# gmh14/tssplat

Measured on AMD Instinct MI355X. Metric: tetrahedra/sec (energy fwd+bwd), higher is better.
Workload: dtype f32

## Files before the change

include/tssplat_amd.h:

```cpp
#ifndef TSSPLAT_AMD_H
#define TSSPLAT_AMD_H

#include <stdint.h>

#ifdef __cplusplus
extern "C" {
#endif

typedef struct tsamd_handle tsamd_handle;

typedef enum tsamd_status {
    TSAMD_OK = 0,
    TSAMD_ERR_INVALID_ARGUMENT = 1,
    TSAMD_ERR_BAD_MESH = 2,
    TSAMD_ERR_NO_DEVICE = 3,
    TSAMD_ERR_HIP = 4,
    TSAMD_ERR_IO = 5,
    TSAMD_ERR_TILING = 6,
    TSAMD_ERR_HOST_ONLY = 7
} tsamd_status;

typedef struct tsamd_options {
    int32_t struct_size;
    int32_t device;
// ... 16 lines not shown
    int64_t total_slots;
    int64_t total_tile_vertices;
    int64_t shared_vertex_copies;
    int64_t finish_vertices;
    int64_t device_bytes;
    int32_t max_slots, max_tile_vertices, block_threads, lds_bytes;
    int32_t slots_per_thread;
    int32_t n_planes;
} tsamd_plan_info;

typedef struct tsamd_tile_view {
    int32_t n_slots, n_owned, s_pad, n_verts, n_excl;
    int64_t stage_off;
    int32_t n_rows;
    int32_t rec_base;
    const uint32_t *planes;
    const uint16_t *row_start;
    const int32_t *gvid;
    const int32_t *vdst;
    const int32_t *slot_tet;
    const float *rest;
} tsamd_tile_view;

const char *tsamd_last_error(void);
const char *tsamd_version(void);
#define TSAMD_ABI_VERSION 3
int32_t tsamd_abi_version(void);

int tsamd_create(const float *rest_xyz, int64_t n_vertices, const int32_t *tets, int64_t n_tets,
                 const tsamd_options *options, tsamd_handle **out);
int tsamd_create_from_veg(const char *path, const tsamd_options *options, tsamd_handle **out);
int tsamd_create_with_operator(const float *rest_xyz, int64_t n_vertices, const int32_t *tets, int64_t n_tets,
                               const int64_t *op_rowptr, const int32_t *op_col, const double *op_val,
                               const tsamd_options *options, tsamd_handle **out);
void tsamd_destroy(tsamd_handle *h);

int64_t tsamd_num_vertices(const tsamd_handle *h);
int64_t tsamd_num_tets(const tsamd_handle *h);
int tsamd_get_plan_info(const tsamd_handle *h, tsamd_plan_info *out);
int tsamd_get_tile(const tsamd_handle *h, int64_t tile, tsamd_tile_view *out);
int tsamd_get_finish_lists(const tsamd_handle *h, int64_t *n_finish, const int32_t **vid,
                           const int32_t **off, const int32_t **idx);
int tsamd_get_adjacency(const tsamd_handle *h, const int32_t **nbr);

int tsamd_forward(tsamd_handle *h, const float *x_dev, float c1, float c2, int order,
                  void *stream, float *energy_dev);
int tsamd_backward(tsamd_handle *h, const float *x_dev, const float *grad_out_dev, float c1, float c2,
                   int order, void *stream, float *grad_dev);
int tsamd_forward_backward(tsamd_handle *h, const float *x_dev, const float *grad_out_dev, float c1,
                           float c2, int order, void *stream, float *energy_dev, float *grad_dev);
int tsamd_evaluate_dev_coef(tsamd_handle *h, const float *x_dev, const float *grad_out_dev, const float *coef_dev,
                            int order, void *stream, float *energy_dev, float *grad_dev);
typedef struct tsamd_graph tsamd_graph;
int tsamd_graph_create(tsamd_handle *h, const float *x_dev, const float *grad_out_dev, int order, float *energy_dev,
                       float *grad_dev, tsamd_graph **out);
int tsamd_graph_launch(tsamd_graph *graph, float c1, float c2, void *stream);
int tsamd_graph_launch_to(tsamd_graph *graph, float c1, float c2, void *stream, float *energy_copy_dev, float *grad_dev);
void tsamd_graph_destroy(tsamd_graph *graph);

typedef struct tsamd_train_loop tsamd_train_loop;
int64_t tsamd_train_loop_workspace_bytes(int32_t n_iters);
int tsamd_train_loop_create(tsamd_handle *h, float *param_dev, float *grad_dev, float *g1_dev, float *g2_dev, float *energy_ring_dev,
                            void *workspace_dev, int32_t n_iters, tsamd_train_loop **out);
// ... 92 lines not shown
```

tssplat_amd/_capi.py:

```python
from __future__ import annotations

import ctypes as C
import os

from . import _build

_lib = None


class TsamdError(RuntimeError):

    def __init__(self, code: int, message: str):
        super().__init__(f"tssplat_amd error {code}: {message}")
        self.code = code


class Options(C.Structure):
    _fields_ = [
        ("struct_size", C.c_int32),
        ("device", C.c_int32),
        ("lds_budget_bytes", C.c_int32),
        ("max_threads", C.c_int32),
        ("target_owned", C.c_int32),
        ("lane_search_sweeps", C.c_int32),
# ... 8 lines not shown

class PlanInfo(C.Structure):
    _fields_ = [
        ("n_vertices", C.c_int64), ("n_tets", C.c_int64), ("n_tiles", C.c_int64),
        ("n_components", C.c_int64), ("total_slots", C.c_int64), ("total_tile_vertices", C.c_int64),
        ("shared_vertex_copies", C.c_int64), ("finish_vertices", C.c_int64), ("device_bytes", C.c_int64),
        ("max_slots", C.c_int32), ("max_tile_vertices", C.c_int32), ("block_threads", C.c_int32),
        ("lds_bytes", C.c_int32), ("slots_per_thread", C.c_int32), ("n_planes", C.c_int32),
    ]

    def as_dict(self) -> dict:
        return {k: int(getattr(self, k)) for k, _ in self._fields_}


class TileView(C.Structure):
    _fields_ = [
        ("n_slots", C.c_int32), ("n_owned", C.c_int32), ("s_pad", C.c_int32), ("n_verts", C.c_int32),
        ("n_excl", C.c_int32), ("stage_off", C.c_int64), ("n_rows", C.c_int32), ("rec_base", C.c_int32),
        ("planes", C.POINTER(C.c_uint32)), ("row_start", C.POINTER(C.c_uint16)),
        ("gvid", C.POINTER(C.c_int32)), ("vdst", C.POINTER(C.c_int32)), ("slot_tet", C.POINTER(C.c_int32)), ("rest", C.POINTER(C.c_float)),
    ]


ABI_VERSION = 3

SIGNATURES = {
    "tsamd_last_error": (C.c_char_p, []),
    "tsamd_version": (C.c_char_p, []),
    "tsamd_abi_version": (C.c_int32, []),
    "tsamd_create": (C.c_int, [C.c_void_p, C.c_int64, C.c_void_p, C.c_int64, C.POINTER(Options), C.POINTER(C.c_void_p)]),
    "tsamd_create_with_operator": (C.c_int, [C.c_void_p, C.c_int64, C.c_void_p, C.c_int64, C.c_void_p, C.c_void_p, C.c_void_p,
                                             C.POINTER(Options), C.POINTER(C.c_void_p)]),
    "tsamd_create_from_veg": (C.c_int, [C.c_char_p, C.POINTER(Options), C.POINTER(C.c_void_p)]),
    "tsamd_destroy": (None, [C.c_void_p]),
    "tsamd_num_vertices": (C.c_int64, [C.c_void_p]),
    "tsamd_num_tets": (C.c_int64, [C.c_void_p]),
    "tsamd_get_plan_info": (C.c_int, [C.c_void_p, C.POINTER(PlanInfo)]),
    "tsamd_get_tile": (C.c_int, [C.c_void_p, C.c_int64, C.POINTER(TileView)]),
    "tsamd_get_finish_lists": (C.c_int, [C.c_void_p, C.POINTER(C.c_int64), C.POINTER(C.POINTER(C.c_int32)),
                                         C.POINTER(C.POINTER(C.c_int32)), C.POINTER(C.POINTER(C.c_int32))]),
    "tsamd_get_adjacency": (C.c_int, [C.c_void_p, C.POINTER(C.POINTER(C.c_int32))]),
    "tsamd_forward": (C.c_int, [C.c_void_p, C.c_void_p, C.c_float, C.c_float, C.c_int, C.c_void_p, C.c_void_p]),
    "tsamd_backward": (C.c_int, [C.c_void_p, C.c_void_p, C.c_void_p, C.c_float, C.c_float, C.c_int, C.c_void_p,
                                 C.c_void_p]),
    "tsamd_forward_backward": (C.c_int, [C.c_void_p, C.c_void_p, C.c_void_p, C.c_float, C.c_float, C.c_int,
                                         C.c_void_p, C.c_void_p, C.c_void_p]),
    "tsamd_evaluate_dev_coef": (C.c_int, [C.c_void_p, C.c_void_p, C.c_void_p, C.c_void_p, C.c_int, C.c_void_p, C.c_void_p,
                                          C.c_void_p]),
    "tsamd_graph_create": (C.c_int, [C.c_void_p, C.c_void_p, C.c_void_p, C.c_int, C.c_void_p, C.c_void_p, C.POINTER(C.c_void_p)]),
    "tsamd_graph_launch": (C.c_int, [C.c_void_p, C.c_float, C.c_float, C.c_void_p]),
    "tsamd_graph_launch_to": (C.c_int, [C.c_void_p, C.c_float, C.c_float, C.c_void_p, C.c_void_p, C.c_void_p]),
    "tsamd_graph_destroy": (None, [C.c_void_p]),
    "tsamd_read_energy_terms": (C.c_int, [C.c_void_p, C.c_void_p, C.POINTER(C.c_double)]),
    "tsamd_set_timing": (C.c_int, [C.c_void_p, C.c_int]),
    "tsamd_get_timing": (C.c_int, [C.c_void_p, C.POINTER(C.c_double), C.POINTER(C.c_double), C.POINTER(C.c_int64)]),
    "tsamd_scale": (C.c_int, [C.c_void_p, C.c_void_p, C.c_void_p, C.c_int64, C.c_void_p]),
    "tsamd_adam_uniform_step": (C.c_int, [C.c_void_p, C.c_void_p, C.c_void_p, C.c_void_p, C.c_int64, C.c_float, C.c_float,
                                        C.c_float, C.c_int64, C.c_float, C.c_void_p, C.c_void_p]),
    "tsamd_grad_limit_workspace_bytes": (C.c_int64, []),
    "tsamd_grad_limit": (C.c_int, [C.c_void_p, C.c_int64, C.c_float, C.c_float, C.c_void_p, C.c_void_p]),
    "tsamd_train_loop_workspace_bytes": (C.c_int64, [C.c_int32]),
# ... 125 lines not shown
```

tssplat_amd/csrc/capi.cpp:

```cpp
#include "../../include/tssplat_amd.h"

#include <hip/hip_runtime_api.h>

#include <algorithm>
#include <cmath>
#include <cstdio>
#include <cstdlib>
#include <cstring>
#include <new>
#include <string>
#include <thread>
#include <vector>

#include "capi_common.h"
#include "kernels.h"
#include "plan.h"

namespace {

thread_local std::string g_err;

int fail(int code, const std::string &msg)
{
    g_err = msg;
// ... 340 lines not shown
    if (!h || !out) return fail(TSAMD_ERR_INVALID_ARGUMENT, "null argument");
    const tsamd::Plan &P = h->plan;
    if (tile < 0 || tile >= int64_t(P.tiles.size())) return fail(TSAMD_ERR_INVALID_ARGUMENT, "tile out of range");
    const tsamd::TileDesc &d = P.tiles[size_t(tile)];
    out->n_slots = d.n_slots;
    out->n_owned = d.n_owned;
    out->s_pad = d.s_pad;
    out->n_verts = d.n_verts;
    out->n_excl = d.n_excl;
    out->stage_off = d.stage_off;
    out->n_rows = d.n_rows;
    out->rec_base = d.rec_base;
    out->planes = P.blob.data() + d.blob_off / 4;
    out->row_start = reinterpret_cast<const uint16_t *>(reinterpret_cast<const uint8_t *>(out->planes) + tsamd::tile_rowtab_offset(P.n_planes, d.s_pad));
    out->gvid = P.gvid.data() + d.vert_off;
    out->vdst = P.vdst.data() + d.vert_off;
    out->slot_tet = P.slot_tet.data() + P.slot_base[size_t(tile)];
    out->rest = P.n_planes == tsamd::kPlanesRebuild
                    ? reinterpret_cast<const float *>(reinterpret_cast<const uint8_t *>(out->planes) + tsamd::tile_rest_offset(P.n_planes, d.s_pad))
                    : nullptr;
    return TSAMD_OK;
}

int tsamd_get_finish_lists(const tsamd_handle *h, int64_t *n_finish, const int32_t **vid, const int32_t **off,
                           const int32_t **idx)
{
    if (!h || !n_finish || !vid || !off || !idx) return fail(TSAMD_ERR_INVALID_ARGUMENT, "null argument");
    *n_finish = int64_t(h->plan.fin_vid.size());
    *vid = h->plan.fin_vid.data();
    *off = h->plan.fin_off.data();
    *idx = h->plan.fin_idx.data();
    return TSAMD_OK;
}

int tsamd_get_adjacency(const tsamd_handle *h, const int32_t **nbr)
{
    if (!h || !nbr) return fail(TSAMD_ERR_INVALID_ARGUMENT, "null argument");
    *nbr = h->plan.nbr.data();
    return TSAMD_OK;
}

int tsamd_forward(tsamd_handle *h, const float *x_dev, float c1, float c2, int order, void *stream,
                  float *energy_dev)
{
    if (!energy_dev) return fail(TSAMD_ERR_INVALID_ARGUMENT, "energy_dev is null");
    return evaluate(h, x_dev, nullptr, c1, c2, order, stream, energy_dev, nullptr);
// ... 221 lines not shown
```

tssplat_amd/csrc/partition.cpp:

```cpp
#include "partition.h"

#include <algorithm>
#include <cmath>

namespace tsamd {
namespace {

constexpr int kLloydIters = 12;
constexpr int kLloydFull = 4;
constexpr int kCandidates = 8;
constexpr int kImproveSweeps = 6;
constexpr int kConnectProbe = 512;
constexpr int64_t kMaxIncidence = int64_t(1) << 23;

inline int64_t copies(int64_t c) { return (c + kMaxRank - 1) / kMaxRank; }

struct Part {
    const Limits &lim;
    int64_t cnt = 0, nv = 0, k = 0;
    std::vector<int32_t> nb;
    std::vector<int32_t> lv;
    std::vector<double> x;
    std::vector<int32_t> part;
    std::vector<int64_t> owned, slots, verts;
    std::vector<int32_t> inc;
    std::vector<int32_t> mark, queue;
    int32_t stamp = 0;

    explicit Part(const Limits &l) : lim(l) {}

    int64_t cost(int64_t p) const { return kPartSlotWeight * slots[size_t(p)] + verts[size_t(p)]; }
    bool fits(int64_t p) const { return lim.fits(slots[size_t(p)], verts[size_t(p)]); }

    void seed(int32_t *idx, int64_t n, int64_t kk, int32_t &next)
    {
        if (kk <= 1) {
            for (int64_t i = 0; i < n; ++i) part[size_t(idx[i])] = next;
            ++next;
            return;
        }
        double lo[3], hi[3];
        for (int d = 0; d < 3; ++d) {
            lo[d] = std::numeric_limits<double>::max();
            hi[d] = -std::numeric_limits<double>::max();
        }
        for (int64_t i = 0; i < n; ++i)
            for (int d = 0; d < 3; ++d) {
                lo[d] = std::min(lo[d], x[3 * size_t(idx[i]) + d]);
                hi[d] = std::max(hi[d], x[3 * size_t(idx[i]) + d]);
            }
        int ax = 0;
        for (int d = 1; d < 3; ++d)
            if (hi[d] - lo[d] > hi[ax] - lo[ax]) ax = d;
        const int64_t k1 = kk / 2;
// ... 5 lines not shown
        seed(idx, mid, k1, next);
        seed(idx + mid, n - mid, kk - k1, next);
    }

    void count_slots(std::vector<int64_t> &s) const
    {
        s.assign(size_t(k), 0);
        for (int64_t q = 0; q < cnt; ++q) {
            const int32_t pq = part[size_t(q)];
            ++s[size_t(pq)];
            int32_t seen[4];
            int ns = 0;
            for (int f = 0; f < 4; ++f) {
                const int32_t r = nb[4 * size_t(q) + f];
                if (r < 0) continue;
                const int32_t pr = part[size_t(r)];
                if (pr == pq || std::find(seen, seen + ns, pr) != seen + ns) continue;
                seen[ns++] = pr;
                ++s[size_t(pr)];
            }
        }
    }

    void lloyd()
    {
        const size_t K = static_cast<size_t>(k);
        std::vector<double> c(3 * K, 0.0), w(K, 0.0), d2c(K);
        std::vector<int64_t> n_in(K), s;
        std::vector<int32_t> cand(K * kCandidates), order(K), next(static_cast<size_t>(cnt));
        const int nc = int(std::min<int64_t>(k, kCandidates));
        for (int it = 0; it < kLloydIters; ++it) {
            std::fill(n_in.begin(), n_in.end(), 0);
            std::vector<double> sum(3 * size_t(k), 0.0);
            for (int64_t e = 0; e < cnt; ++e) {
                const int32_t p = part[size_t(e)];
                ++n_in[size_t(p)];
                for (int d = 0; d < 3; ++d) sum[3 * size_t(p) + d] += x[3 * size_t(e) + d];
            }
            for (int64_t p = 0; p < k; ++p)
                if (n_in[size_t(p)] > 0)
                    for (int d = 0; d < 3; ++d) c[3 * size_t(p) + d] = sum[3 * size_t(p) + d] / double(n_in[size_t(p)]);
            count_slots(s);
            double r2 = 0.0;
            for (int64_t e = 0; e < cnt; ++e) {
                const int32_t p = part[size_t(e)];
                for (int d = 0; d < 3; ++d) {
                    const double t = x[3 * size_t(e) + d] - c[3 * size_t(p) + d];
                    r2 += t * t;
                }
            }
            r2 /= double(std::max<int64_t>(1, cnt));
            int64_t s_sum = 0, live = 0;
            for (int64_t p = 0; p < k; ++p)
                if (n_in[size_t(p)] > 0) {
                    s_sum += s[size_t(p)];
                    ++live;
                }
            const double s_mean = double(s_sum) / double(std::max<int64_t>(1, live));
            for (int64_t p = 0; p < k; ++p) w[size_t(p)] += 0.5 * r2 * (s_mean - double(s[size_t(p)])) / s_mean;
            for (int64_t p = 0; p < k; ++p) {
                for (int64_t q = 0; q < k; ++q) {
                    double d = 0.0;
                    for (int dd = 0; dd < 3; ++dd) {
                        const double t = c[3 * size_t(q) + dd] - c[3 * size_t(p) + dd];
                        d += t * t;
// ... 8 lines not shown
            }
            for (int64_t e = 0; e < cnt; ++e) {
                const int32_t p = part[size_t(e)];
                next[size_t(e)] = p;
                if (it >= kLloydFull && in_cell(int32_t(e), p) == faces(int32_t(e))) continue;
                int32_t best = p;
                double best_d = std::numeric_limits<double>::max();
                for (int j = 0; j < nc; ++j) {
                    const int32_t q = cand[size_t(p) * kCandidates + size_t(j)];
                    double d = -w[size_t(q)];
                    for (int dd = 0; dd < 3; ++dd) {
                        const double t = x[3 * size_t(e) + dd] - c[3 * size_t(q) + dd];
                        d += t * t;
                    }
                    if (d < best_d || (d == best_d && q < best)) {
                        best_d = d;
                        best = q;
                    }
                }
                next[size_t(e)] = best;
            }
            part.swap(next);
        }
    }

    void connect()
    {
        std::vector<int32_t> piece(size_t(cnt), -1), best_piece(size_t(k), -1);
        std::vector<int64_t> piece_size;
        for (int64_t s0 = 0; s0 < cnt; ++s0) {
            if (piece[size_t(s0)] >= 0) continue;
            const int32_t id = int32_t(piece_size.size()), p = part[size_t(s0)];
            queue.assign(1, int32_t(s0));
            piece[size_t(s0)] = id;
            for (size_t h = 0; h < queue.size(); ++h)
                for (int f = 0; f < 4; ++f) {
                    const int32_t r = nb[4 * size_t(queue[h]) + f];
                    if (r < 0 || piece[size_t(r)] >= 0 || part[size_t(r)] != p) continue;
                    piece[size_t(r)] = id;
                    queue.push_back(r);
                }
            piece_size.push_back(int64_t(queue.size()));
            if (best_piece[size_t(p)] < 0 || piece_size[size_t(best_piece[size_t(p)])] < int64_t(queue.size())) best_piece[size_t(p)] = id;
        }
        int64_t left = 0;
        for (int64_t e = 0; e < cnt; ++e)
// ... 112 lines not shown
    int64_t vert_delta(int32_t p, const int32_t *t, int n, int sign) const
    {
        int32_t vs[20], ds[20];
        int m = 0;
        for (int i = 0; i < n; ++i)
            for (int a = 0; a < 4; ++a) {
                const int32_t v = lv[4 * size_t(t[i]) + a];
                int j = int(std::find(vs, vs + m, v) - vs);
                if (j == m) {
                    vs[m] = v;
                    ds[m++] = 0;
                }
                ds[j] += sign;
            }
        int64_t d = 0;
        for (int j = 0; j < m; ++j) {
            const int32_t c = inc[size_t(p) * size_t(nv) + size_t(vs[j])];
            d += copies(c + ds[j]) - copies(c);
        }
        return d;
    }
    struct Move {
        int32_t e = -1, B = -1;
        int64_t dcost = 0, key = 0;
        int nl = 0, ne = 0;
        int32_t gone[5], en[4];
        int64_t dsA = 0, dvA = 0, dsB = 0, dvB = 0;
    };
    bool evaluate(int32_t e, int32_t B, Move &mv) const
    {
        const int32_t A = part[size_t(e)];
        mv.e = e;
        mv.B = B;
        mv.nl = leaving(e, A, mv.gone);
        mv.ne = entering(e, B, mv.en);
        mv.dsA = -mv.nl;
        mv.dsB = mv.ne;
        mv.dvB = vert_delta(B, mv.en, mv.ne, +1);
        if (!lim.fits(slots[size_t(B)] + mv.dsB, verts[size_t(B)] + mv.dvB)) return false;
        mv.dvA = vert_delta(A, mv.gone, mv.nl, -1);
        mv.dcost = kPartSlotWeight * (mv.dsA + mv.dsB) + mv.dvA + mv.dvB;
        return true;
    }
    void apply(const Move &mv)
    {
        const int32_t A = part[size_t(mv.e)];
        for (int i = 0; i < mv.nl; ++i) remove_slot(A, mv.gone[i]);
        for (int i = 0; i < mv.ne; ++i) add_slot(mv.B, mv.en[i]);
        part[size_t(mv.e)] = mv.B;
        --owned[size_t(A)];
        ++owned[size_t(mv.B)];
    }
    bool stays_connected(int32_t e)
    {
        const int32_t A = part[size_t(e)];
        int32_t want[4];
        int nw = 0;
        for (int f = 0; f < 4; ++f) {
            const int32_t q = nb[4 * size_t(e) + f];
            if (q >= 0 && part[size_t(q)] == A && std::find(want, want + nw, q) == want + nw) want[nw++] = q;
        }
        if (nw <= 1) return true;
        if (++stamp == std::numeric_limits<int32_t>::max()) {
            std::fill(mark.begin(), mark.end(), 0);
// ... 24 lines not shown
            if (pq != A && std::find(out, out + n, pq) == out + n) out[n++] = pq;
        }
        return n;
    }

    bool repair()
    {
        std::vector<int32_t> members;
        for (int64_t A = 0; A < k; ++A) {
            if (fits(A)) continue;
            members.clear();
            for (int64_t e = 0; e < cnt; ++e)
                if (part[size_t(e)] == A) members.push_back(int32_t(e));
            while (!fits(A)) {
                if (owned[size_t(A)] <= 1) return false;
                Move best, mv;
                bool have = false;
                for (int32_t e : members) {
                    if (part[size_t(e)] != A) continue;
                    int32_t oc[4];
                    const int no = other_cells(e, oc);
                    for (int j = 0; j < no; ++j) {
                        if (!evaluate(e, oc[j], mv)) continue;
                        mv.key = mv.dcost + kPartSlotWeight * mv.dsA + mv.dvA;
                        if (have && mv.key >= best.key) continue;
                        if (!stays_connected(e)) break;
                        best = mv;
                        have = true;
                    }
                }
                if (!have) return false;
                apply(best);
            }
        }
        return true;
    }

    void improve()
    {
        for (int sweep = 0; sweep < kImproveSweeps; ++sweep) {
            int64_t moved = 0;
            for (int64_t e = 0; e < cnt; ++e) {
                const int32_t A = part[size_t(e)];
                if (owned[size_t(A)] <= 1) continue;
                int32_t oc[4];
                const int no = other_cells(int32_t(e), oc);
                Move best, mv;
                bool have = false;
                for (int j = 0; j < no; ++j) {
                    if (!evaluate(int32_t(e), oc[j], mv) || mv.dcost >= 0) continue;
                    if (have && mv.dcost >= best.dcost) continue;
                    best = mv;
                    have = true;
                }
                if (have && stays_connected(int32_t(e))) {
                    apply(best);
                    ++moved;
                }
            }
            if (moved == 0) break;
        }
    }
};

}

bool partition_component(const Mesh &M, const Limits &lim, const float *cen, const int32_t *ids, int64_t cnt,
                         int64_t k_first, int64_t k_last, Scratch &S, std::vector<std::vector<int32_t>> &parts,
                         int64_t &cost)
{
    parts.clear();
    cost = 0;
    k_first = std::max<int64_t>(2, k_first);
    k_last = std::min(k_last, cnt);
    if (k_first > k_last) return false;
    Part P(lim);
    P.cnt = cnt;
    P.nb.resize(4 * size_t(cnt));
    P.lv.resize(4 * size_t(cnt));
    P.x.resize(3 * size_t(cnt));
    const int32_t st = S.next();
    for (int64_t i = 0; i < cnt; ++i) {
        S.tet_stamp[size_t(ids[i])] = st;
        S.tet_slot[size_t(ids[i])] = int32_t(i);
    }
    for (int64_t i = 0; i < cnt; ++i) {
        const int64_t g = ids[i];
        for (int f = 0; f < 4; ++f) {
            const int32_t q = M.nbr[4 * g + f];
            P.nb[4 * size_t(i) + f] = q >= 0 && S.tet_stamp[size_t(q)] == st ? S.tet_slot[size_t(q)] : -1;
            const int32_t v = M.tets[4 * g + f];
            if (S.vert_stamp[size_t(v)] != st) {
                S.vert_stamp[size_t(v)] = st;
                S.vert_local[size_t(v)] = int32_t(P.nv++);
            }
            P.lv[4 * size_t(i) + f] = S.vert_local[size_t(v)];
        }
        for (int d = 0; d < 3; ++d) P.x[3 * size_t(i) + d] = cen[3 * size_t(g) + d];
    }
    if (k_last * P.nv > kMaxIncidence) return false;
    P.mark.assign(size_t(cnt), 0);
    std::vector<int32_t> idx(static_cast<size_t>(cnt));
    for (int64_t k = k_first; k <= k_last; ++k) {
        P.k = k;
        P.part.assign(size_t(cnt), 0);
        for (int64_t i = 0; i < cnt; ++i) idx[size_t(i)] = int32_t(i);
        int32_t next = 0;
        P.seed(idx.data(), cnt, k, next);
        P.lloyd();
        P.connect();
        P.build_state();
        if (!P.repair()) continue;
        P.improve();
        std::vector<int64_t> at(size_t(k), -1);
        for (int64_t p = 0; p < k; ++p)
            if (P.owned[size_t(p)] > 0) {
                at[size_t(p)] = int64_t(parts.size());
                parts.emplace_back();
                parts.back().reserve(size_t(P.owned[size_t(p)]));
                cost += P.cost(p);
            }
        for (int64_t i = 0; i < cnt; ++i) parts[size_t(at[size_t(P.part[size_t(i)])])].push_back(ids[i]);
        return true;
    }
    return false;
}

}
```

tssplat_amd/csrc/partition.h:

```cpp
#pragma once

#include "plan.h"

#include <cstdint>
#include <limits>
#include <vector>

namespace tsamd {

struct Scratch {
    std::vector<int32_t> tet_stamp, tet_slot, vert_stamp, vert_local;
    int32_t stamp = 0;
    void init(int64_t m, int64_t n)
    {
        if (int64_t(tet_stamp.size()) != m) {
            tet_stamp.assign(size_t(m), 0);
            tet_slot.assign(size_t(m), 0);
        }
        if (int64_t(vert_stamp.size()) != n) {
            vert_stamp.assign(size_t(n), 0);
            vert_local.assign(size_t(n), 0);
        }
    }
    int32_t next()
    {
        if (stamp > std::numeric_limits<int32_t>::max() - 8) {
// ... 8 lines not shown

struct Limits {
    int64_t budget;
    int64_t max_spad;
    int64_t pad_unit = 4;
    bool rebuild = false;
    bool fits(int64_t n_slots, int64_t n_verts) const
    {
        const int64_t sp = (n_slots + pad_unit - 1) / pad_unit * pad_unit;
        return sp <= max_spad && n_verts <= kMaxTileVerts && tile_lds_bytes(sp, n_verts, rebuild) <= budget;
    }
};

struct Mesh {
    const float *rest;
    const int32_t *tets;
    const int32_t *nbr;
    int64_t n, m;
};

void measure(const Mesh &M, const int32_t *owned, int64_t cnt, Scratch &S, int64_t &n_slots, int64_t &n_verts,
             std::vector<int32_t> *halo_out = nullptr);

constexpr int64_t kPartSlotWeight = 3;

bool partition_component(const Mesh &M, const Limits &lim, const float *cen, const int32_t *ids, int64_t cnt,
                         int64_t k_first, int64_t k_last, Scratch &S, std::vector<std::vector<int32_t>> &parts,
                         int64_t &cost);

}
```

tssplat_amd/csrc/plan.cpp:

```cpp
#include "plan.h"

#include "conflict_opt.h"
#include "partition.h"

#include <algorithm>
#include <atomic>
#include <cmath>
#include <cstdio>
#include <cstdlib>
#include <cstring>
#include <fstream>
#include <functional>
#include <limits>
#include <numeric>
#include <sstream>
#include <chrono>
#include <thread>

namespace tsamd {
namespace {

struct StageTimer {
    bool on = std::getenv("TSAMD_PLAN_TIMING") != nullptr;
    std::chrono::steady_clock::time_point t0 = std::chrono::steady_clock::now();
    void lap(const char *what)
    {
        if (!on) return;
        const auto t1 = std::chrono::steady_clock::now();
        std::fprintf(stderr, "[plan] %-28s %8.3f s\n", what, std::chrono::duration<double>(t1 - t0).count());
        t0 = t1;
    }
};

enum { OK = 0, ERR_INVALID = 1, ERR_BAD_MESH = 2, ERR_IO = 5, ERR_TILING = 6 };

template <class Fn>
void parallel_chunks(int64_t n, int64_t chunk, int nthreads, Fn fn)
{
    if (n <= 0) return;
    nthreads = std::max(1, nthreads);
    if (nthreads == 1 || n <= chunk) {
        fn(int64_t(0), n, 0);
        return;
    }
    std::atomic<int64_t> next{0};
    auto body = [&](int worker) {
        for (;;) {
            int64_t b = next.fetch_add(chunk, std::memory_order_relaxed);
            if (b >= n) break;
            fn(b, std::min(n, b + chunk), worker);
        }
    };
    std::vector<std::thread> pool;
    for (int t = 1; t < nthreads; ++t) pool.emplace_back(body, t);
    body(0);
    for (auto &th : pool) th.join();
}
// ... 229 lines not shown
    int nthreads = opt.num_threads > 0 ? std::min(opt.num_threads, 64) : std::min(int(std::thread::hardware_concurrency()), 32);
    nthreads = std::max(1, nthreads);
    const int spt = opt.slots_per_lane > 0 ? opt.slots_per_lane : kSlotsPerLane;
    if (spt < 2 || spt > 4) {
        err = "slots_per_lane must be 2, 3 or 4";
        return ERR_INVALID;
    }
    if (opt.max_threads > 1024) {
        err = "max_threads exceeds 1024";
        return ERR_INVALID;
    }
    int max_threads = opt.max_threads > 0 ? opt.max_threads : kTileThreads;
    max_threads = std::max(64, (max_threads / 64) * 64);
    Limits lim;
    lim.budget = opt.lds_budget > 0 ? opt.lds_budget : 80 * 1024;
    lim.pad_unit = spt == 3 ? 12 : 4;
    lim.max_spad = int64_t(spt) * int64_t(max_threads) / lim.pad_unit * lim.pad_unit;
    lim.rebuild = opt.rebuild_dminv != 0 && op == nullptr;
    if (lim.budget < tile_lds_bytes(12, 8, lim.rebuild)) {
        err = "lds_budget_bytes too small";
        return ERR_INVALID;
    }

    P = Plan();
    P.n = n;
    P.m = m;
    P.spt = spt;
    int rc = build_adjacency(tets, n, m, P.nbr, nthreads, err);
    if (rc) return rc;
    Mesh M{rest, tets, P.nbr.data(), n, m};
    timer.lap("face adjacency");

    if (op) {
        if (!op->rowptr || (m > 0 && op->rowptr[m] > 0 && (!op->col || !op->val))) {
            err = "element operator: null CSR array";
            return ERR_INVALID;
        }
        if (op->rowptr[0] != 0 || op->rowptr[m] < 0) {
            err = "element operator: rowptr[0] must be 0 and rowptr[m] non-negative";
            return ERR_INVALID;
        }
        if (opt.rebuild_dminv) {
            err = "element operator: not combined with rebuild_dminv (the explicit-operator kernels stream Dm^-1)";
            return ERR_INVALID;
        }
        P.n_planes = kPlanesWeighted;
        P.op_diag.assign(size_t(m), 0.f);
        P.op_w.assign(size_t(4 * m), 0.f);
        std::vector<double> dg(static_cast<size_t>(m), 0.0), w(static_cast<size_t>(4 * m), 0.0);
        for (int64_t e = 0; e < m; ++e) {
// ... 193 lines not shown
                    sp.split(ids, cnt, k);
                    done = !sp.failed && !sp.rc;
                    k = std::max<int64_t>(k + 1, (k * 103 + 99) / 100);
                }
                if (!done) group_tiles[size_t(g)].clear();
                group_fitted[size_t(g)] = done ? 1 : 0;
            }
            sp.strict = false;
            sp.failed = false;
            if (!done) sp.split(ids, cnt, (cnt + target - 1) / target);
            if (sp.rc) {
                first_rc.store(sp.rc);
                bool expected = false;
                if (err_set.compare_exchange_strong(expected, true)) split_err = local_err;
            }
        }
    });
    if (first_rc.load()) {
        err = split_err;
        return first_rc.load();
    }

    timer.lap("bisection");
    std::vector<int64_t> rcb_slots(groups.size(), 0), rcb_cost(groups.size(), 0), rcb_lds(groups.size(), 0);
    parallel_chunks(int64_t(groups.size()), 16, nthreads, [&](int64_t b, int64_t e, int w) {
        Scratch &S = get_scratch(w);
        for (int64_t g = b; g < e; ++g)
            for (const auto &l : group_tiles[size_t(g)]) {
                int64_t ns, nv;
                measure(M, l.data(), int64_t(l.size()), S, ns, nv);
                rcb_slots[size_t(g)] += ns;
                rcb_cost[size_t(g)] += kPartSlotWeight * ns + nv;
                const int64_t sp = (ns + lim.pad_unit - 1) / lim.pad_unit * lim.pad_unit;
                rcb_lds[size_t(g)] = std::max(rcb_lds[size_t(g)], tile_lds_bytes(sp, nv, rebuild));
            }
    });
    Limits cell_lim = lim;
    cell_lim.budget = 0;
    for (int64_t l : rcb_lds) cell_lim.budget = std::max(cell_lim.budget, std::min(lim.budget, l));
    std::atomic<int64_t> n_cut{0}, n_refined{0};
    parallel_chunks(int64_t(groups.size()), 1, nthreads, [&](int64_t b, int64_t e, int w) {
        Scratch &S = get_scratch(w);
        std::vector<std::vector<int32_t>> parts;
        for (int64_t g = b; g < e; ++g) {
            if (!group_fitted[size_t(g)]) continue;
            const Group &G = groups[size_t(g)];
            const int32_t *ids = comp_tets.data() + comp_start[G.cb];
            const int64_t cnt = comp_start[G.ce] - comp_start[G.cb];
            auto &leaves = group_tiles[size_t(g)];
            const int64_t k_rcb = int64_t(leaves.size());
            n_cut.fetch_add(1, std::memory_order_relaxed);
            const int64_t k_lo = (rcb_slots[size_t(g)] + s_cap - 1) / s_cap;
            int64_t cost;
            if (!partition_component(M, cell_lim, cen.data(), ids, cnt, k_lo, std::min(k_rcb, k_lo + 3), S, parts, cost)) continue;
            if (int64_t(parts.size()) > k_rcb || (int64_t(parts.size()) == k_rcb && cost >= rcb_cost[size_t(g)])) continue;
            n_refined.fetch_add(1, std::memory_order_relaxed);
            leaves.clear();
            std::string unused_err;
            Splitter sp{M, lim, cen, S, leaves, unused_err};
            for (auto &part : parts) sp.emit(part.data(), int64_t(part.size()));
        }
    });
    if (timer.on)
        std::fprintf(stderr, "[plan] partition: %lld cut components, %lld refined, %lld keep the bisection\n", (long long)n_cut.load(),
                     (long long)n_refined.load(), (long long)(n_cut.load() - n_refined.load()));
    timer.lap("partition (cells + refinement)");
    std::vector<std::vector<int32_t>> tiles_owned;
    for (auto &gt : group_tiles)
        for (auto &t : gt) tiles_owned.push_back(std::move(t));
    group_tiles.clear();
    const int64_t T = int64_t(tiles_owned.size());

    std::vector<std::vector<int32_t>> tile_halo(static_cast<size_t>(T)), tile_verts(static_cast<size_t>(T)), tile_vdeg(static_cast<size_t>(T));
    std::vector<std::atomic<int32_t>> vcount(static_cast<size_t>(n));
    for (auto &a : vcount) a.store(0, std::memory_order_relaxed);
    parallel_chunks(T, 4, nthreads, [&](int64_t b, int64_t e, int w) {
        Scratch &S = get_scratch(w);
        std::vector<int32_t> uniq, cnt;
        std::vector<std::pair<int32_t, int32_t>> key;
        for (int64_t t = b; t < e; ++t) {
            const auto &own = tiles_owned[size_t(t)];
            int64_t ns, nv;
            measure(M, own.data(), int64_t(own.size()), S, ns, nv, &tile_halo[size_t(t)]);
            uniq.clear();
            cnt.clear();
            const int32_t st = S.next();
            auto touch = [&](int32_t el) {
                for (int a = 0; a < 4; ++a) {
                    const int32_t v = tets[4 * int64_t(el) + a];
// ... 46 lines not shown
        int32_t n_excl = 0;
        for (int32_t v : tv) n_excl += vcount[size_t(v)].load(std::memory_order_relaxed) == 1;
        d.n_owned = int32_t(tiles_owned[size_t(t)].size());
        d.n_slots = d.n_owned + int32_t(tile_halo[size_t(t)].size());
        d.s_pad = int32_t((d.n_slots + lim.pad_unit - 1) / lim.pad_unit * lim.pad_unit);
        d.n_verts = int32_t(tv.size());
        d.n_excl = n_excl;
        d.blob_off = uint64_t(blob_bytes);
        d.vert_off = int32_t(vert_off);
        d.stage_off = stage_off;
        d.n_rows = tv.empty() ? 0 : tile_vdeg[size_t(t)][0];
        d.rec_base = int32_t(tile_rec_base(d.n_verts, rebuild));
        if (d.n_verts > kMaxTileVerts || 4 * int64_t(d.s_pad) > 65535) {
            err = "tile exceeds the 10-bit vertex / 16-bit entry fields of the plan";
            return ERR_TILING;
        }
        blob_bytes += (tile_rest_offset(n_planes, d.s_pad) + (rebuild ? 16 * int64_t(d.n_verts) : 0) + 127) & ~int64_t(127);
        vert_off += vert_stride;
        P.total_tile_verts += d.n_verts;
        stage_off += d.n_verts - d.n_excl;
        P.slot_base[size_t(t)] = slot_off;
        slot_off += d.s_pad;
        P.total_slots += d.n_slots;
        P.max_slots = std::max(P.max_slots, d.n_slots);
        P.max_verts = std::max(P.max_verts, d.n_verts);
        P.lds_bytes = std::max<int32_t>(P.lds_bytes, int32_t(tile_lds_bytes(d.s_pad, d.n_verts, rebuild)));
        max_quads = std::max(max_quads, d.s_pad / spt);
        if (vert_off >= (int64_t(1) << 31)) {
            err = "too many tile vertices for 32-bit offsets";
            return ERR_TILING;
        }
    }
    P.slot_base[size_t(T)] = slot_off;
    P.n_stage = stage_off;
    P.block_threads = std::min(max_threads, ((max_quads + 63) / 64) * 64);
    P.blob.resize(size_t(blob_bytes / 4));
    P.gvid.resize(size_t(vert_off));
    P.vdst.resize(size_t(vert_off));
    P.slot_tet.resize(size_t(slot_off));

    std::vector<int32_t> fin_of(static_cast<size_t>(n), -1);
    {
        int64_t entries = 0;
        for (int64_t v = 0; v < n; ++v) {
            int32_t c = vcount[size_t(v)].load(std::memory_order_relaxed);
            if (c == 1) continue;
// ... 400 lines not shown
```

tssplat_amd/csrc/plan.h:

```cpp
#pragma once

#include <cstdint>
#include <memory>
#include <string>
#include <utility>
#include <vector>

#ifdef __HIPCC__
#define TSAMD_HOST_DEVICE __host__ __device__
#else
#define TSAMD_HOST_DEVICE
#endif

namespace tsamd {

struct PlanOptions {
    int lds_budget = 0;
    int max_threads = 0;
    int target_owned = 0;
    int num_threads = 0;
    int conflict_aware = 1;
    int lane_search_sweeps = 2;
    int rebuild_dminv = 0;
    int slots_per_lane = 0;
};

struct TileDesc {
    uint64_t blob_off;
    int32_t n_slots;
    int32_t n_owned;
    int32_t s_pad;
    int32_t n_verts;
    int32_t n_excl;
    int32_t vert_off;
    int64_t stage_off;
    int32_t n_rows;
    int32_t rec_base;
};
static_assert(sizeof(TileDesc) == 48, "TileDesc layout is part of the kernel ABI");

constexpr int kPlanes = 13;
constexpr int kRowTabEntries = 72;
constexpr int kMaxRank = 64;
constexpr int kSlotsPerLane = 2;
constexpr int kTileThreads = 768;
constexpr int kPlanesWeighted = 22;
constexpr int kPlanesWeightedSym = 18;
constexpr int kPlanesRebuild = 4;
// ... 50 lines not shown
        else
            ::new (static_cast<void *>(p)) U(std::forward<Args>(args)...);
    }
};
template <class T>
using RawVector = std::vector<T, DefaultInitAllocator<T>>;

struct Plan {
    int64_t n = 0, m = 0;
    int64_t n_components = 0;
    std::vector<int32_t> nbr;
    std::vector<TileDesc> tiles;
    RawVector<uint32_t> blob;
    RawVector<int32_t> gvid;
    RawVector<int32_t> vdst;
    RawVector<int32_t> slot_tet;
    std::vector<int64_t> slot_base;
    std::vector<int32_t> fin_vid, fin_off, fin_idx;
    int64_t n_stage = 0;
    int64_t total_slots = 0, total_tile_verts = 0;
    int32_t max_slots = 0, max_verts = 0, block_threads = 64, lds_bytes = 0, spt = kSlotsPerLane;
    int32_t n_planes = kPlanes;
    int32_t vert_stride = 64;
    std::vector<float> op_diag;
    std::vector<float> op_w;
};

struct ElementOperatorCSR {
    const int64_t *rowptr;
    const int32_t *col;
    const double *val;
};

int build_plan(const float *rest, int64_t n, const int32_t *tets, int64_t m, const PlanOptions &opt,
               Plan &plan, std::string &err, const ElementOperatorCSR *op = nullptr);

int build_adjacency(const int32_t *tets, int64_t n, int64_t m, std::vector<int32_t> &nbr, int nthreads,
                    std::string &err);

int read_veg(const char *path, std::vector<float> &rest, std::vector<int32_t> &tets, std::string &err);

}
```

tssplat_amd/tet_spheres_ext.py:

```python
from __future__ import annotations

import contextlib
import ctypes as C
import os
import sys

import numpy as np
import torch

from . import _capi

__all__ = ["TetSpheres", "forward", "backward", "random_x", "grad_limit"]

_lib = _capi.load()
CPU_ENERGY = os.environ.get("TSSPLAT_AMD_CPU_ENERGY", "0") == "1"
REBUILD_DMINV = {"1": 1, "2": 2}.get(os.environ.get("TSSPLAT_AMD_REBUILD_DMINV", "0"), 0)
print("initializing")


_raw_stream = getattr(torch._C, "_cuda_getCurrentRawStream", None)


def _stream_ptr(device: torch.device) -> int:
    if _raw_stream is not None and device.index is not None:
# ... 74 lines not shown
        self.nele = int(_lib.tsamd_num_tets(self._h))
        self.n3 = 3 * self.n

    def close(self) -> None:
        if getattr(self, "_h", None) is not None and self._h.value:
            _lib.tsamd_destroy(self._h)
            self._h = C.c_void_p()
        self._cache = None

    def __del__(self):
        try:
            self.close()
        except Exception:
            pass

    def _handle(self):
        if not self._h.value:
            raise RuntimeError("TetSpheres object is empty (construction failed or it was closed)")
        return self._h

    def plan_info(self) -> dict:
        info = _capi.PlanInfo()
        _capi.check(_lib.tsamd_get_plan_info(self._handle(), C.byref(info)))
        return info.as_dict()

    def set_timing(self, enable: bool) -> None:
        _capi.check(_lib.tsamd_set_timing(self._handle(), int(enable)))

    def get_timing(self) -> tuple[float, float, int]:
        a, b, n = C.c_double(), C.c_double(), C.c_int64()
        _capi.check(_lib.tsamd_get_timing(self._handle(), C.byref(a), C.byref(b), C.byref(n)))
        return a.value, b.value, n.value

    def energy_terms(self) -> tuple[float, float]:
        out = (C.c_double * 2)()
        _capi.check(_lib.tsamd_read_energy_terms(self._handle(), _stream_ptr(self.device), out))
        return float(out[0]), float(out[1])


def _check_input(x: torch.Tensor, ts: TetSpheres) -> torch.Tensor:
    if not isinstance(x, torch.Tensor):
        raise TypeError("input must be a torch.Tensor")
    if not x.is_cuda:
        raise RuntimeError("tssplat_amd: input must live on the GPU; there is no CPU fallback")
    if ts.device is None or x.device != ts.device:
        raise RuntimeError(f"input is on {x.device} but the TetSpheres object lives on {ts.device}")
    if x.dtype != torch.float32:
# ... 72 lines not shown
```

Baseline: 58.57 billion.

## Drive tet partitioning with a wavefront-aware modelled tile cost

Replaces the linear slot/vertex partition cost with a fitted model that charges per tile, per 64-lane wave slot, per slot and per vertex. Local move evaluation, refinement acceptance and the cell-versus-bisection choice all use this model. It also raises the Lloyd iteration count, widens the range of tile counts searched, and adds early rejection of over-capacity candidates. A partition-mode option and an info query are added. The goal is a tiling whose tiles waste fewer partially filled waves in the kernel, at the price of more planning time and dependence on fitted constants.

```diff
diff --git a/include/tssplat_amd.h b/include/tssplat_amd.h
--- a/include/tssplat_amd.h
+++ b/include/tssplat_amd.h
@@ -62,6 +62,14 @@
     const float *rest;
 } tsamd_tile_view;
 
+typedef struct tsamd_partition_info {
+    int32_t struct_size;
+    int32_t mode;
+    int64_t cut_components;
+    int64_t cell_components;
+    double modelled_tile_cost;
+} tsamd_partition_info;
+
 const char *tsamd_last_error(void);
 const char *tsamd_version(void);
 #define TSAMD_ABI_VERSION 3
@@ -79,6 +87,7 @@
 int64_t tsamd_num_tets(const tsamd_handle *h);
 int tsamd_get_plan_info(const tsamd_handle *h, tsamd_plan_info *out);
 int tsamd_get_tile(const tsamd_handle *h, int64_t tile, tsamd_tile_view *out);
+int tsamd_get_partition_info(const tsamd_handle *h, tsamd_partition_info *out);
 int tsamd_get_finish_lists(const tsamd_handle *h, int64_t *n_finish, const int32_t **vid,
                            const int32_t **off, const int32_t **idx);
 int tsamd_get_adjacency(const tsamd_handle *h, const int32_t **nbr);
diff --git a/tssplat_amd/_capi.py b/tssplat_amd/_capi.py
--- a/tssplat_amd/_capi.py
+++ b/tssplat_amd/_capi.py
@@ -54,6 +54,14 @@
     ]
 
 
+class PartitionInfo(C.Structure):
+    _fields_ = [("struct_size", C.c_int32), ("mode", C.c_int32), ("cut_components", C.c_int64), ("cell_components", C.c_int64),
+                ("modelled_tile_cost", C.c_double)]
+
+
+PARTITION_MODES = ("auto", "bisection", "cells")
+
+
 ABI_VERSION = 3
 
 SIGNATURES = {
@@ -69,6 +77,7 @@
     "tsamd_num_tets": (C.c_int64, [C.c_void_p]),
     "tsamd_get_plan_info": (C.c_int, [C.c_void_p, C.POINTER(PlanInfo)]),
     "tsamd_get_tile": (C.c_int, [C.c_void_p, C.c_int64, C.POINTER(TileView)]),
+    "tsamd_get_partition_info": (C.c_int, [C.c_void_p, C.POINTER(PartitionInfo)]),
     "tsamd_get_finish_lists": (C.c_int, [C.c_void_p, C.POINTER(C.c_int64), C.POINTER(C.POINTER(C.c_int32)),
                                          C.POINTER(C.POINTER(C.c_int32)), C.POINTER(C.POINTER(C.c_int32))]),
     "tsamd_get_adjacency": (C.c_int, [C.c_void_p, C.POINTER(C.POINTER(C.c_int32))]),
diff --git a/tssplat_amd/csrc/capi.cpp b/tssplat_amd/csrc/capi.cpp
--- a/tssplat_amd/csrc/capi.cpp
+++ b/tssplat_amd/csrc/capi.cpp
@@ -386,6 +386,22 @@
     return TSAMD_OK;
 }
 
+int tsamd_get_partition_info(const tsamd_handle *h, tsamd_partition_info *out)
+{
+    if (!h || !out) return fail(TSAMD_ERR_INVALID_ARGUMENT, "null argument");
+    if (out->struct_size < int32_t(2 * sizeof(int32_t)) || out->struct_size > int32_t(sizeof(tsamd_partition_info)))
+        return fail(TSAMD_ERR_INVALID_ARGUMENT, "tsamd_partition_info: set struct_size to sizeof(tsamd_partition_info)");
+    tsamd_partition_info info;
+    std::memset(&info, 0, sizeof(info));
+    info.struct_size = out->struct_size;
+    info.mode = h->plan.partition_mode;
+    info.cut_components = h->plan.n_cut;
+    info.cell_components = h->plan.n_cells;
+    info.modelled_tile_cost = h->plan.tile_cost;
+    std::memcpy(out, &info, size_t(out->struct_size));
+    return TSAMD_OK;
+}
+
 int tsamd_get_finish_lists(const tsamd_handle *h, int64_t *n_finish, const int32_t **vid, const int32_t **off,
                            const int32_t **idx)
 {
diff --git a/tssplat_amd/csrc/partition.cpp b/tssplat_amd/csrc/partition.cpp
--- a/tssplat_amd/csrc/partition.cpp
+++ b/tssplat_amd/csrc/partition.cpp
@@ -2,14 +2,16 @@
 
 #include <algorithm>
 #include <cmath>
+#include <numeric>
 
 namespace tsamd {
 namespace {
 
-constexpr int kLloydIters = 12;
+constexpr int kLloydIters = 40;
 constexpr int kLloydFull = 4;
 constexpr int kCandidates = 8;
 constexpr int kImproveSweeps = 6;
+constexpr double kMinGain = 1e-9;
 constexpr int kConnectProbe = 512;
 constexpr int64_t kMaxIncidence = int64_t(1) << 23;
 
@@ -17,6 +19,7 @@
 
 struct Part {
     const Limits &lim;
+    const int spt;
     int64_t cnt = 0, nv = 0, k = 0;
     std::vector<int32_t> nb;
     std::vector<int32_t> lv;
@@ -27,9 +30,10 @@
     std::vector<int32_t> mark, queue;
     int32_t stamp = 0;
 
-    explicit Part(const Limits &l) : lim(l) {}
-
-    int64_t cost(int64_t p) const { return kPartSlotWeight * slots[size_t(p)] + verts[size_t(p)]; }
+    Part(const Limits &l, int slots_per_lane) : lim(l), spt(slots_per_lane) {}
+
+    double cost_of(int64_t o, int64_t s, int64_t v) const { return o > 0 ? tile_cost(o, s, v, lim.pad_unit, spt) : 0.0; }
+    double cost(int64_t p) const { return cost_of(owned[size_t(p)], slots[size_t(p)], verts[size_t(p)]); }
     bool fits(int64_t p) const { return lim.fits(slots[size_t(p)], verts[size_t(p)]); }
 
     void seed(int32_t *idx, int64_t n, int64_t kk, int32_t &next)
@@ -81,7 +85,7 @@
         }
     }
 
-    void lloyd()
+    bool lloyd()
     {
         const size_t K = static_cast<size_t>(k);
         std::vector<double> c(3 * K, 0.0), w(K, 0.0), d2c(K);
@@ -100,6 +104,7 @@
                 if (n_in[size_t(p)] > 0)
                     for (int d = 0; d < 3; ++d) c[3 * size_t(p) + d] = sum[3 * size_t(p) + d] / double(n_in[size_t(p)]);
             count_slots(s);
+            if (it == kLloydFull && std::accumulate(s.begin(), s.end(), int64_t(0)) > k * lim.max_spad) return false;
             double r2 = 0.0;
             for (int64_t e = 0; e < cnt; ++e) {
                 const int32_t p = part[size_t(e)];
@@ -154,6 +159,7 @@
             }
             part.swap(next);
         }
+        return true;
     }
 
     void connect()
@@ -312,7 +318,7 @@
     }
     struct Move {
         int32_t e = -1, B = -1;
-        int64_t dcost = 0, key = 0;
+        double dcost = 0, dcostA = 0, key = 0;
         int nl = 0, ne = 0;
         int32_t gone[5], en[4];
         int64_t dsA = 0, dvA = 0, dsB = 0, dvB = 0;
@@ -329,7 +335,9 @@
         mv.dvB = vert_delta(B, mv.en, mv.ne, +1);
         if (!lim.fits(slots[size_t(B)] + mv.dsB, verts[size_t(B)] + mv.dvB)) return false;
         mv.dvA = vert_delta(A, mv.gone, mv.nl, -1);
-        mv.dcost = kPartSlotWeight * (mv.dsA + mv.dsB) + mv.dvA + mv.dvB;
+        const size_t a = size_t(A), b = size_t(B);
+        mv.dcostA = cost_of(owned[a] - 1, slots[a] + mv.dsA, verts[a] + mv.dvA) - cost(A);
+        mv.dcost = mv.dcostA + cost_of(owned[b] + 1, slots[b] + mv.dsB, verts[b] + mv.dvB) - cost(B);
         return true;
     }
     void apply(const Move &mv)
@@ -400,7 +408,7 @@
                     const int no = other_cells(e, oc);
                     for (int j = 0; j < no; ++j) {
                         if (!evaluate(e, oc[j], mv)) continue;
-                        mv.key = mv.dcost + kPartSlotWeight * mv.dsA + mv.dvA;
+                        mv.key = mv.dcost + mv.dcostA;
                         if (have && mv.key >= best.key) continue;
                         if (!stays_connected(e)) break;
                         best = mv;
@@ -426,7 +434,7 @@
                 Move best, mv;
                 bool have = false;
                 for (int j = 0; j < no; ++j) {
-                    if (!evaluate(int32_t(e), oc[j], mv) || mv.dcost >= 0) continue;
+                    if (!evaluate(int32_t(e), oc[j], mv) || mv.dcost > -kMinGain) continue;
                     if (have && mv.dcost >= best.dcost) continue;
                     best = mv;
                     have = true;
@@ -443,16 +451,16 @@
 
 }
 
-bool partition_component(const Mesh &M, const Limits &lim, const float *cen, const int32_t *ids, int64_t cnt,
+bool partition_component(const Mesh &M, const Limits &lim, int spt, const float *cen, const int32_t *ids, int64_t cnt,
                          int64_t k_first, int64_t k_last, Scratch &S, std::vector<std::vector<int32_t>> &parts,
-                         int64_t &cost)
+                         double &cost)
 {
     parts.clear();
     cost = 0;
     k_first = std::max<int64_t>(2, k_first);
     k_last = std::min(k_last, cnt);
     if (k_first > k_last) return false;
-    Part P(lim);
+    Part P(lim, spt);
     P.cnt = cnt;
     P.nb.resize(4 * size_t(cnt));
     P.lv.resize(4 * size_t(cnt));
@@ -485,9 +493,10 @@
         for (int64_t i = 0; i < cnt; ++i) idx[size_t(i)] = int32_t(i);
         int32_t next = 0;
         P.seed(idx.data(), cnt, k, next);
-        P.lloyd();
+        if (!P.lloyd()) continue;
         P.connect();
         P.build_state();
+        if (std::accumulate(P.slots.begin(), P.slots.end(), int64_t(0)) > k * lim.max_spad) continue;
         if (!P.repair()) continue;
         P.improve();
         std::vector<int64_t> at(size_t(k), -1);
diff --git a/tssplat_amd/csrc/partition.h b/tssplat_amd/csrc/partition.h
--- a/tssplat_amd/csrc/partition.h
+++ b/tssplat_amd/csrc/partition.h
@@ -2,6 +2,7 @@
 
 #include "plan.h"
 
+#include <algorithm>
 #include <cstdint>
 #include <limits>
 #include <vector>
@@ -56,10 +57,37 @@
 void measure(const Mesh &M, const int32_t *owned, int64_t cnt, Scratch &S, int64_t &n_slots, int64_t &n_verts,
              std::vector<int32_t> *halo_out = nullptr);
 
-constexpr int64_t kPartSlotWeight = 3;
+struct TileFeatures {
+    int64_t wave_slots, owned_wave_slots;
+};
+inline TileFeatures tile_features(int64_t n_owned, int64_t n_slots, int64_t pad_unit, int spt)
+{
+    const int64_t s_pad = (n_slots + pad_unit - 1) / pad_unit * pad_unit, nq = s_pad / spt;
+    TileFeatures f{0, 0};
+    for (int p = 0; p < spt; ++p) {
+        const int64_t filled = std::max<int64_t>(0, std::min(nq, n_slots - p * nq));
+        const int64_t owned = std::max<int64_t>(0, std::min(nq, n_owned - p * nq));
+        f.wave_slots += (filled + 63) / 64;
+        f.owned_wave_slots += (owned + 63) / 64;
+    }
+    return f;
+}
+constexpr double kCostTile = 3.21 + 0.77;
+constexpr double kCostWaveSlot = 0.176;
+constexpr double kCostSlot = 0.0009;
+constexpr double kCostVert = 0.0007;
+inline double tile_cost(int64_t n_owned, int64_t n_slots, int64_t n_verts, int64_t pad_unit, int spt)
+{
+    const TileFeatures f = tile_features(n_owned, n_slots, pad_unit, spt);
+    return kCostTile + kCostWaveSlot * double(f.wave_slots) + kCostSlot * double(n_slots) + kCostVert * double(n_verts);
+}
 
-bool partition_component(const Mesh &M, const Limits &lim, const float *cen, const int32_t *ids, int64_t cnt,
+constexpr double kMinCellGain = 0.005;
+
+constexpr double kCellSlotGain = 0.94;
+
+bool partition_component(const Mesh &M, const Limits &lim, int spt, const float *cen, const int32_t *ids, int64_t cnt,
                          int64_t k_first, int64_t k_last, Scratch &S, std::vector<std::vector<int32_t>> &parts,
-                         int64_t &cost);
+                         double &cost);
 
 }
diff --git a/tssplat_amd/csrc/plan.cpp b/tssplat_amd/csrc/plan.cpp
--- a/tssplat_amd/csrc/plan.cpp
+++ b/tssplat_amd/csrc/plan.cpp
@@ -33,6 +33,16 @@
 };
 
 enum { OK = 0, ERR_INVALID = 1, ERR_BAD_MESH = 2, ERR_IO = 5, ERR_TILING = 6 };
+
+int partition_mode_from_env(std::string &err)
+{
+    const char *v = std::getenv("TSAMD_PARTITION");
+    if (!v || !*v || !std::strcmp(v, "auto")) return kPartitionAuto;
+    if (!std::strcmp(v, "bisection")) return kPartitionBisection;
+    if (!std::strcmp(v, "cells")) return kPartitionCells;
+    err = std::string("TSAMD_PARTITION must be bisection, cells or auto, got '") + v + "'";
+    return -1;
+}
 
 template <class Fn>
 void parallel_chunks(int64_t n, int64_t chunk, int nthreads, Fn fn)
@@ -308,10 +318,17 @@
         return ERR_INVALID;
     }
 
+    const int part_mode = opt.partition >= 0 ? opt.partition : partition_mode_from_env(err);
+    if (part_mode < kPartitionAuto || part_mode > kPartitionCells) {
+        if (err.empty()) err = "partition must be -1 (environment), 0 (auto), 1 (bisection) or 2 (cells)";
+        return ERR_INVALID;
+    }
+
     P = Plan();
     P.n = n;
     P.m = m;
     P.spt = spt;
+    P.partition_mode = part_mode;
     int rc = build_adjacency(tets, n, m, P.nbr, nthreads, err);
     if (rc) return rc;
     Mesh M{rest, tets, P.nbr.data(), n, m};
@@ -551,7 +568,8 @@
     }
 
     timer.lap("bisection");
-    std::vector<int64_t> rcb_slots(groups.size(), 0), rcb_cost(groups.size(), 0), rcb_lds(groups.size(), 0);
+    std::vector<int64_t> rcb_slots(groups.size(), 0), rcb_lds(groups.size(), 0);
+    std::vector<double> rcb_cost(groups.size(), 0.0);
     parallel_chunks(int64_t(groups.size()), 16, nthreads, [&](int64_t b, int64_t e, int w) {
         Scratch &S = get_scratch(w);
         for (int64_t g = b; g < e; ++g)
@@ -559,7 +577,7 @@
                 int64_t ns, nv;
                 measure(M, l.data(), int64_t(l.size()), S, ns, nv);
                 rcb_slots[size_t(g)] += ns;
-                rcb_cost[size_t(g)] += kPartSlotWeight * ns + nv;
+                rcb_cost[size_t(g)] += tile_cost(int64_t(l.size()), ns, nv, lim.pad_unit, spt);
                 const int64_t sp = (ns + lim.pad_unit - 1) / lim.pad_unit * lim.pad_unit;
                 rcb_lds[size_t(g)] = std::max(rcb_lds[size_t(g)], tile_lds_bytes(sp, nv, rebuild));
             }
@@ -573,16 +591,18 @@
         std::vector<std::vector<int32_t>> parts;
         for (int64_t g = b; g < e; ++g) {
             if (!group_fitted[size_t(g)]) continue;
+            n_cut.fetch_add(1, std::memory_order_relaxed);
+            if (part_mode == kPartitionBisection) continue;
             const Group &G = groups[size_t(g)];
             const int32_t *ids = comp_tets.data() + comp_start[G.cb];
             const int64_t cnt = comp_start[G.ce] - comp_start[G.cb];
             auto &leaves = group_tiles[size_t(g)];
             const int64_t k_rcb = int64_t(leaves.size());
-            n_cut.fetch_add(1, std::memory_order_relaxed);
-            const int64_t k_lo = (rcb_slots[size_t(g)] + s_cap - 1) / s_cap;
-            int64_t cost;
-            if (!partition_component(M, cell_lim, cen.data(), ids, cnt, k_lo, std::min(k_rcb, k_lo + 3), S, parts, cost)) continue;
-            if (int64_t(parts.size()) > k_rcb || (int64_t(parts.size()) == k_rcb && cost >= rcb_cost[size_t(g)])) continue;
+            const int64_t k_lo = int64_t(std::ceil(kCellSlotGain * double(rcb_slots[size_t(g)]) / double(s_cap)));
+            const int64_t k_hi = std::min(k_rcb, (rcb_slots[size_t(g)] + s_cap - 1) / s_cap + 3);
+            double cost;
+            if (!partition_component(M, cell_lim, spt, cen.data(), ids, cnt, k_lo, k_hi, S, parts, cost)) continue;
+            if (part_mode == kPartitionAuto && cost >= (1.0 - kMinCellGain) * rcb_cost[size_t(g)]) continue;
             n_refined.fetch_add(1, std::memory_order_relaxed);
             leaves.clear();
             std::string unused_err;
@@ -594,6 +614,8 @@
         std::fprintf(stderr, "[plan] partition: %lld cut components, %lld refined, %lld keep the bisection\n", (long long)n_cut.load(),
                      (long long)n_refined.load(), (long long)(n_cut.load() - n_refined.load()));
     timer.lap("partition (cells + refinement)");
+    P.n_cut = n_cut.load();
+    P.n_cells = n_refined.load();
     std::vector<std::vector<int32_t>> tiles_owned;
     for (auto &gt : group_tiles)
         for (auto &t : gt) tiles_owned.push_back(std::move(t));
@@ -686,6 +708,7 @@
         P.slot_base[size_t(t)] = slot_off;
         slot_off += d.s_pad;
         P.total_slots += d.n_slots;
+        P.tile_cost += tile_cost(d.n_owned, d.n_slots, d.n_verts, lim.pad_unit, spt);
         P.max_slots = std::max(P.max_slots, d.n_slots);
         P.max_verts = std::max(P.max_verts, d.n_verts);
         P.lds_bytes = std::max<int32_t>(P.lds_bytes, int32_t(tile_lds_bytes(d.s_pad, d.n_verts, rebuild)));
diff --git a/tssplat_amd/csrc/plan.h b/tssplat_amd/csrc/plan.h
--- a/tssplat_amd/csrc/plan.h
+++ b/tssplat_amd/csrc/plan.h
@@ -23,7 +23,9 @@
     int lane_search_sweeps = 2;
     int rebuild_dminv = 0;
     int slots_per_lane = 0;
+    int partition = -1;
 };
+enum { kPartitionAuto = 0, kPartitionBisection = 1, kPartitionCells = 2 };
 
 struct TileDesc {
     uint64_t blob_off;
@@ -120,6 +122,9 @@
     int32_t max_slots = 0, max_verts = 0, block_threads = 64, lds_bytes = 0, spt = kSlotsPerLane;
     int32_t n_planes = kPlanes;
     int32_t vert_stride = 64;
+    int32_t partition_mode = kPartitionAuto;
+    int64_t n_cut = 0, n_cells = 0;
+    double tile_cost = 0.0;
     std::vector<float> op_diag;
     std::vector<float> op_w;
 };
diff --git a/tssplat_amd/tet_spheres_ext.py b/tssplat_amd/tet_spheres_ext.py
--- a/tssplat_amd/tet_spheres_ext.py
+++ b/tssplat_amd/tet_spheres_ext.py
@@ -120,7 +120,10 @@
     def plan_info(self) -> dict:
         info = _capi.PlanInfo()
         _capi.check(_lib.tsamd_get_plan_info(self._handle(), C.byref(info)))
-        return info.as_dict()
+        part = _capi.PartitionInfo(struct_size=C.sizeof(_capi.PartitionInfo))
+        _capi.check(_lib.tsamd_get_partition_info(self._handle(), C.byref(part)))
+        return dict(info.as_dict(), partition=_capi.PARTITION_MODES[part.mode], cut_components=int(part.cut_components),
+                    cell_components=int(part.cell_components), modelled_tile_cost_us=float(part.modelled_tile_cost))
 
     def set_timing(self, enable: bool) -> None:
         _capi.check(_lib.tsamd_set_timing(self._handle(), int(enable)))
```

Result: no change. 58.98 billion (median of 6 runs) (+0.7%).
